# suvajit-patra/sl-hwgat

Hardware: AMD Instinct MI355X
Metric: clips/sec fwd+bwd at B=64 T=128 J=67; %HBM roofline; 1->8 GPU scaling (higher is better)
Workload: dtype f32

## Files before the change

### sl-hwgat_amd/csrc/gemm_f32.h

```cpp
#pragma once
#include "common.h"

struct NtArgs {
    const float* A; const float* W; const float* bias; float* C;
    float* C2; const float* res; const float* aux;
    const float* mean; const float* rstd; const float* gamma; const float* beta;
    int64_t M; int N, K;
    uint32_t pro_seed, epi_seed; float pro_p, epi_p;
    int64_t row0;
    float* stat_sum; float* stat_sq;
    int mg_F, mg_K;
    const uint32_t* seed_base;
};

struct MergeWalk {
    int k, f; int64_t b; int F, K, step;
    __device__ __forceinline__ void start(int64_t m, int F_, int K_, int step_) {
        F = F_; K = K_; step = step_;
        const uint32_t mm = (uint32_t)m, fr = mm / (uint32_t)K_;
        k = (int)(mm - fr * (uint32_t)K_);
        const uint32_t bb = fr / (uint32_t)F_;
        f = (int)(fr - bb * (uint32_t)F_);
        b = bb;
    }
    __device__ __forceinline__ int64_t mrow() const { return (b * (F >> 1) + (f >> 1)) * K + k; }
    __device__ __forceinline__ int64_t off(int N) const { return mrow() * (2 * (int64_t)N) + (int64_t)(f & 1) * N; }
    __device__ __forceinline__ void next() {
        k += step;
        const bool wk = k >= K;
        k -= wk ? K : 0;
        f += wk ? 1 : 0;
        const bool wf = f >= F;
        f -= wf ? F : 0;
        b += wf ? 1 : 0;
    }
};

struct TnArgs {
    const float* A; const float* B; float* dW; float* db;
    const float* mean; const float* rstd; const float* gamma; const float* beta;
    int64_t M; int N, K;
    int n_split; int64_t rows_per_split;
    uint32_t pro_seed; float pro_p;
    int64_t row0;
    const uint32_t* seed_base;
    float* det_dw; float* det_db; int det_cap;
};


int hwgat_launch_tn256(TnArgs a, hipStream_t st, float* ws = nullptr, int64_t ws_floats = 0);
int64_t hwgat_tn256_ws_floats(int64_t M, int N, int K);

int hwgat_launch_nt256(const NtArgs& a, int pro, int epi, hipStream_t st);
```

### sl-hwgat_amd/csrc/gemm_f32.hip

```cpp
#include <stdlib.h>
#include <type_traits>
#include "common.h"
#include "fused_ops.h"
#include "gemm_f32.h"
#include "gemm_tn64.h"

namespace {

constexpr int BK_MIN = 16;

using NtSmall = TileCfg<2, 2, 2, 2>;
using NtBig = TileCfg<4, 2, 2, 4, 32, 1>;
using NtK16 = TileCfg<2, 2, 2, 2, 16, 3>;
using NtN64 = TileCfg<4, 1, 1, 2>;

template <int PRO, int EPI, typename C, bool RAGGED = false, int STAT = 0>
__global__ __launch_bounds__(C::THREADS, C::OCC * C::THREADS / 256) void gemm_nt_k(NtArgs p) {
    HWGAT_RESOLVE_SEEDS2(p);
    constexpr int BM = C::BM, BN = C::BN, TMW = C::TMW, TNW = C::TNW, PA = C::PA, PW = C::PW, RPP = C::RPP;
    constexpr int BK = C::BK, LDT = C::LDT;
    __shared__ __attribute__((aligned(16))) float sm[2 * (BM + BN) * LDT];
    const int tid = threadIdx.x, lane = tid & 63, wave = tid >> 6;
    const int lq = lane & 31, hh = lane >> 5;
    const int wm = wave / C::WN, wn = wave % C::WN;
// ... 230 lines not shown
                        }
                    }
                    __builtin_amdgcn_fence(__ATOMIC_ACQ_REL, "wavefront");
                    __builtin_amdgcn_wave_barrier();
                }
            }
            if constexpr (STAT == X_STAT || STAT == X_STAT_MERGE) {
                __syncthreads();
                for (int q = tid; q < BM; q += C::THREADS) {
                    int64_t mr = m0 + q;
                    if constexpr (STAT == X_STAT_MERGE) { MergeWalk w; w.start(m0 + q, p.mg_F, p.mg_K, 1); mr = w.mrow(); }
                    atomicAdd(p.stat_sum + mr, rowstat[2 * q]);
                    atomicAdd(p.stat_sq + mr, rowstat[2 * q + 1]);
                }
            }
        }
        __syncthreads();
        t += gridDim.x;
        if (t >= n_tiles) break;
        m0 = mn; n0 = nn;
    }
}


using TnSmall = TileCfg<2, 2, 2, 2>;
using TnBig = TileCfg<4, 2, 2, 4, 32, 1>;
using TnK16 = TileCfg<2, 2, 2, 2, 16, 3>;

template <int PRO, bool BLN, typename C, bool MF16 = false, bool RAGGED = false>
__global__ __launch_bounds__(C::THREADS, C::OCC * C::THREADS / 256) void gemm_tn_k(TnArgs p) {
    HWGAT_RESOLVE_SEED1(p);
    constexpr int TM = C::BK;
    constexpr int BT = C::BM;
    constexpr int LDR = MF16 ? BT + 16 : BT;
    constexpr int TNW = C::TMW, TKW = C::TNW;
    constexpr int TPR = BT / 4;
    constexpr int RPP = C::THREADS / TPR;
    constexpr int NP = TM / RPP;
    __shared__ __attribute__((aligned(16))) float sm[2 * 2 * TM * LDR];
    const int tid = threadIdx.x, lane = tid & 63, wave = tid >> 6;
    const int lq = lane & 31, hh = lane >> 5;
    const int wn = wave / C::WN, wk = wave % C::WN;
    const int tiles_n = p.N / BT, tiles_k = p.K / BT, n_tiles = tiles_n * tiles_k;
    const int xcd = blockIdx.x & 7, j = blockIdx.x >> 3;
    const int tile = j % n_tiles;
    const int split = (j / n_tiles) * 8 + xcd;
    if (split >= p.n_split) return;
    const int n0 = (tile / tiles_k) * BT, k0 = (tile % tiles_k) * BT;
    const int64_t r_begin = (int64_t)split * p.rows_per_split;
    const int64_t r_end = r_begin + p.rows_per_split < p.M ? r_begin + p.rows_per_split : p.M;
    if (r_begin >= r_end) return;
    const int n_it = RAGGED ? (int)((r_end - r_begin + TM - 1) / TM) : (int)((r_end - r_begin) / TM);
    const int64_t m_last = p.M - 1;

    const int lrow = tid / TPR, lc4 = (tid % TPR) * 4;
    const uint32_t pro_th = drop_thresh(p.pro_p);
    const float pro_sc = 1.0f / (1.0f - p.pro_p);
    f32x4 ra[NP], rb[NP];
    float bm[NP], bs[NP];
    f32x4 colsum = {0.f, 0.f, 0.f, 0.f};
    f32x4 lg = {1.f, 1.f, 1.f, 1.f}, lb = {0.f, 0.f, 0.f, 0.f};
    if constexpr (BLN) {
        lg = *reinterpret_cast<const f32x4*>(p.gamma + k0 + lc4);
        lb = *reinterpret_cast<const f32x4*>(p.beta + k0 + lc4);
    }

    auto issue = [&](int it) {
        const int64_t r0 = r_begin + (int64_t)it * TM + lrow;
#pragma unroll
        for (int i = 0; i < NP; ++i) {
            int64_t row = r0 + RPP * i;
            if constexpr (RAGGED) row = row < m_last ? row : m_last;
            ra[i] = *reinterpret_cast<const f32x4*>(p.A + row * p.N + n0 + lc4);
            rb[i] = *reinterpret_cast<const f32x4*>(p.B + row * p.K + k0 + lc4);
            if constexpr (BLN) { bm[i] = p.mean[row]; bs[i] = p.rstd[row]; }
        }
    };
    auto commit = [&](int buf, int it) {
        float* As = sm + buf * (2 * TM * LDR);
        float* Bs = As + TM * LDR;
        const int64_t r0 = r_begin + (int64_t)it * TM + lrow;
#pragma unroll
        for (int i = 0; i < NP; ++i) {
            f32x4 a = ra[i], b = rb[i];
            if constexpr (PRO == PRO_DROP)
                a *= drop_keep4(p.pro_seed, (uint64_t)((RAGGED ? p.row0 : 0) + r0 + RPP * i) * p.N + n0 + lc4, pro_th, pro_sc);
            if constexpr (BLN) b = (b - bm[i]) * bs[i] * lg + lb;
            if constexpr (RAGGED) { if (r0 + RPP * i > m_last) a = f32x4{0.f, 0.f, 0.f, 0.f}; }
            colsum += a;
            *reinterpret_cast<f32x4*>(As + (lrow + RPP * i) * LDR + lc4) = a;
            *reinterpret_cast<f32x4*>(Bs + (lrow + RPP * i) * LDR + lc4) = b;
        }
    };

    constexpr int TI = MF16 ? TNW * 2 : TNW, TJ = MF16 ? TKW * 2 : TKW, TS = MF16 ? 16 : 32;
    typedef typename std::conditional<MF16, f32x4, f32x16>::type acc_t;
    acc_t acc[TI][TJ];
#pragma unroll
    for (int i = 0; i < TI; ++i)
#pragma unroll
        for (int jj = 0; jj < TJ; ++jj)
#pragma unroll
            for (int e = 0; e < (MF16 ? 4 : 16); ++e) acc[i][jj][e] = 0.f;

    issue(0);
    commit(0, 0);
    __syncthreads();
    int buf = 0;
    const int lc = MF16 ? (lane & 15) : lq, lk = MF16 ? (lane >> 4) : hh;
    constexpr int KPS = MF16 ? 4 : 2;
    for (int it = 0; it < n_it; ++it) {
        const bool have_next = it + 1 < n_it;
        if (have_next) issue(it + 1);
        const float* As = sm + buf * (2 * TM * LDR) + wn * (TNW * 32) + lc;
        const float* Bs = sm + buf * (2 * TM * LDR) + TM * LDR + wk * (TKW * 32) + lc;
        constexpr int NSTEP = TM / KPS, CH = MF16 ? 2 : 4, NCH = NSTEP / CH;
        float fa[2][CH][TI], fb[2][CH][TJ];
        auto fetch = [&](int c, int slot) {
#pragma unroll
            for (int e = 0; e < CH; ++e) {
                const int ro = (KPS * (c * CH + e) + lk) * LDR;
#pragma unroll
                for (int i = 0; i < TI; ++i) fa[slot][e][i] = As[ro + TS * i];
#pragma unroll
                for (int jj = 0; jj < TJ; ++jj) fb[slot][e][jj] = Bs[ro + TS * jj];
            }
        };
        fetch(0, 0);
#pragma unroll
        for (int c = 0; c < NCH; ++c) {
            if (c + 1 < NCH) fetch(c + 1, (c + 1) & 1);
            __builtin_amdgcn_sched_barrier(0);
#pragma unroll
            for (int e = 0; e < CH; ++e)
#pragma unroll
                for (int i = 0; i < TI; ++i)
#pragma unroll
                    for (int jj = 0; jj < TJ; ++jj) {
                        if constexpr (MF16)
                            acc[i][jj] = __builtin_amdgcn_mfma_f32_16x16x4f32(fa[c & 1][e][i], fb[c & 1][e][jj], acc[i][jj], 0, 0, 0);
                        else
                            acc[i][jj] = __builtin_amdgcn_mfma_f32_32x32x2f32(fa[c & 1][e][i], fb[c & 1][e][jj], acc[i][jj], 0, 0, 0);
                    }
            __builtin_amdgcn_sched_barrier(0);
        }
        if (have_next) commit(buf ^ 1, it + 1);
        __syncthreads();
        buf ^= 1;
    }
    const bool det = p.det_dw != nullptr;
    float* dwo = det ? p.det_dw + (int64_t)split * p.N * p.K : p.dW;
#pragma unroll
    for (int i = 0; i < TI; ++i)
#pragma unroll
        for (int jj = 0; jj < TJ; ++jj)
#pragma unroll
            for (int r = 0; r < (MF16 ? 4 : 16); ++r) {
                const int n = n0 + wn * (TNW * 32) + i * TS + (MF16 ? 4 * lk + r : crow(r, hh));
                const int k = k0 + wk * (TKW * 32) + jj * TS + lc;
                HWGAT_TN_ACC(det, dwo, (int64_t)n * p.K + k, acc[i][jj][r]);
            }
    if (p.db != nullptr && k0 == 0) {
        float* red = sm;
        __syncthreads();
        *reinterpret_cast<f32x4*>(red + lrow * BT + lc4) = colsum;
        __syncthreads();
        if (tid < BT) {
            float s = 0.f;
#pragma unroll
            for (int q = 0; q < RPP; ++q) s += red[q * BT + tid];
            HWGAT_TN_ACC(det, det ? p.det_db + (int64_t)split * p.N : p.db, n0 + tid, s);
        }
    }
}

__global__ void transpose_k(const float* __restrict__ in, float* __restrict__ out, int R, int C) {
    __shared__ float tile[32][33];
    const int c0 = blockIdx.x * 32, r0 = blockIdx.y * 32;
    for (int i = threadIdx.y; i < 32; i += 8)
        if (r0 + i < R && c0 + threadIdx.x < C) tile[i][threadIdx.x] = in[(int64_t)(r0 + i) * C + c0 + threadIdx.x];
    __syncthreads();
    for (int i = threadIdx.y; i < 32; i += 8)
        if (c0 + i < C && r0 + threadIdx.x < R) out[(int64_t)(c0 + i) * R + r0 + threadIdx.x] = tile[threadIdx.x][i];
}

template <int PRO, typename C, bool RAGGED = false>
int launch_nt(const NtArgs& a, int epi, hipStream_t st, bool fold = false) {
    const int64_t tiles = ((a.M + C::BM - 1) / C::BM) * (a.N / C::BN);
    const int grid = (int)(tiles < C::SLOTS ? tiles : C::SLOTS);
    if (fold) {
        if constexpr (PRO == PRO_NONE) {
            if (epi == EPI_BIAS) gemm_nt_k<PRO_NONE, EPI_BIAS, C, RAGGED, X_LNFOLD><<<grid, C::THREADS, 0, st>>>(a);
            else if (epi == EPI_BIAS_GELU_DROP) gemm_nt_k<PRO_NONE, EPI_BIAS_GELU_DROP, C, RAGGED, X_LNFOLD><<<grid, C::THREADS, 0, st>>>(a);
            else if (epi == EPI_BIAS_GELU_DROP_G) gemm_nt_k<PRO_NONE, EPI_BIAS_GELU_DROP_G, C, RAGGED, X_LNFOLD><<<grid, C::THREADS, 0, st>>>(a);
            else return HWGAT_EINVAL;
            HWGAT_LAUNCH_CHECK();
        }
        return HWGAT_EINVAL;
    }
    if (a.stat_sum != nullptr) {
        if constexpr (PRO == PRO_NONE && !RAGGED) {
            if (a.mg_K > 0) gemm_nt_k<PRO_NONE, EPI_BIAS_DROP_RES, C, false, 2><<<grid, C::THREADS, 0, st>>>(a);
            else gemm_nt_k<PRO_NONE, EPI_BIAS_DROP_RES, C, false, 1><<<grid, C::THREADS, 0, st>>>(a);
            HWGAT_LAUNCH_CHECK();
        }
        return HWGAT_EINVAL;
    }
    switch (epi) {
        case EPI_BIAS: gemm_nt_k<PRO, EPI_BIAS, C, RAGGED><<<grid, C::THREADS, 0, st>>>(a); break;
        case EPI_BIAS_DROP_RES: gemm_nt_k<PRO, EPI_BIAS_DROP_RES, C, RAGGED><<<grid, C::THREADS, 0, st>>>(a); break;
        case EPI_BIAS_GELU_DROP: gemm_nt_k<PRO, EPI_BIAS_GELU_DROP, C, RAGGED><<<grid, C::THREADS, 0, st>>>(a); break;
        case EPI_GELU_BWD: gemm_nt_k<PRO, EPI_GELU_BWD, C, RAGGED><<<grid, C::THREADS, 0, st>>>(a); break;
        case EPI_BIAS_GELU_DROP_G: gemm_nt_k<PRO, EPI_BIAS_GELU_DROP_G, C, RAGGED><<<grid, C::THREADS, 0, st>>>(a); break;
        case EPI_MUL_AUX: gemm_nt_k<PRO, EPI_MUL_AUX, C, RAGGED><<<grid, C::THREADS, 0, st>>>(a); break;
        case EPI_NONE: gemm_nt_k<PRO, EPI_NONE, C, RAGGED><<<grid, C::THREADS, 0, st>>>(a); break;
        case EPI_BIAS_RELU_DROP:
            if constexpr (PRO == PRO_NONE) { gemm_nt_k<PRO_NONE, EPI_BIAS_RELU_DROP, C, RAGGED><<<grid, C::THREADS, 0, st>>>(a); break; }
            return HWGAT_EINVAL;
        case EPI_RELU_BWD:
            if constexpr (PRO == PRO_NONE) { gemm_nt_k<PRO_NONE, EPI_RELU_BWD, C, RAGGED><<<grid, C::THREADS, 0, st>>>(a); break; }
            return HWGAT_EINVAL;
        default: return HWGAT_EINVAL;
    }
    HWGAT_LAUNCH_CHECK();
}

NtArgs nt_rows(NtArgs a, int64_t r0, int64_t rows) {
    a.A += r0 * a.K;
    a.C += r0 * a.N;
    if (a.C2) a.C2 += r0 * a.N;
    if (a.res) a.res += r0 * a.N;
    if (a.aux) a.aux += r0 * a.N;
    if (a.mean) { a.mean += r0; a.rstd += r0; }
    a.M = rows;
    a.row0 = r0;
    return a;
}
TnArgs tn_rows(TnArgs a, int64_t r0, int64_t rows) {
    a.A += r0 * a.N;
    a.B += r0 * a.K;
    if (a.mean) { a.mean += r0; a.rstd += r0; }
    a.M = rows;
    a.row0 = r0;
    return a;
}

int tile_override() {
    static const int v = [] {
        const char* e = lab_env("HWGAT_GEMM_TILE");
        return !e ? 0 : (e[0] == 's' ? 1 : (e[0] == 'b' ? 2 : (e[0] == 'k' ? 3 : (e[0] == 'm' ? 6 : (e[0] == 't' ? 7 : 0)))));
    }();
    return v;
}

int launch_nt_n64(const NtArgs& a, int pro, int epi, hipStream_t st) {
    const int64_t m_bulk = a.M / 128 * 128;
    if (m_bulk) {
        NtArgs b = a;
        b.M = m_bulk;
        int rc;
        switch (pro) {
            case PRO_NONE: rc = launch_nt<PRO_NONE, NtN64>(b, epi, st); break;
            case PRO_LN_FOLD: rc = launch_nt<PRO_NONE, NtN64>(b, epi, st, true); break;
            case PRO_LN: rc = launch_nt<PRO_LN, NtN64>(b, epi, st); break;
            case PRO_DROP: rc = launch_nt<PRO_DROP, NtN64>(b, epi, st); break;
            default: return HWGAT_EINVAL;
        }
        if (rc || m_bulk == a.M) return rc;
    }
    const NtArgs t = nt_rows(a, m_bulk, a.M - m_bulk);
    switch (pro) {
        case PRO_NONE: return launch_nt<PRO_NONE, NtN64, true>(t, epi, st);
        case PRO_LN: return launch_nt<PRO_LN, NtN64, true>(t, epi, st);
        case PRO_DROP: return launch_nt<PRO_DROP, NtN64, true>(t, epi, st);
        default: return HWGAT_EINVAL;
    }
}

template <int PRO, bool BLN, typename C, bool MF16 = false, bool RAGGED = false>
int launch_tn(TnArgs a, hipStream_t st) {
    constexpr int TM = C::BK;
    const int n_tiles = (a.N / C::BM) * (a.K / C::BM);
    auto gcd = [](int x, int y) { while (y) { int t = x % y; x = y; y = t; } return x; };
    const int r_min = n_tiles / gcd(n_tiles, C::SLOTS);
    static const int min_rounds = [] { const char* e = lab_env("HWGAT_TN_ROUNDS"); return e ? atoi(e) : 1; }();
    int r = r_min;
    while (r < min_rounds) r += r_min;
    int64_t want = (int64_t)C::SLOTS * r / n_tiles;
    const int64_t max_split = a.M / (TM * 16) > 0 ? a.M / (TM * 16) : 1;
    if (want > max_split) want = max_split;
    if (want < 1) want = 1;
    int64_t rows = (a.M + want - 1) / want;
    rows = (rows + TM - 1) / TM * TM;
    a.n_split = (int)((a.M + rows - 1) / rows);
    a.rows_per_split = rows;
    if (a.det_dw && a.n_split > a.det_cap) return HWGAT_ESHAPE;
    const int grid = ((a.n_split + 7) / 8) * 8 * n_tiles;
    gemm_tn_k<PRO, BLN, C, MF16, RAGGED><<<grid, C::THREADS, 0, st>>>(a);
    HWGAT_LAUNCH_CHECK();
}

}

extern "C" int hwgat_linear_nt_f32_ex(const float* A, const float* W, const float* bias, float* C, int64_t M,
                                      int N, int K, int pro, const float* mean, const float* rstd,
                                      const float* gamma, const float* beta, uint32_t pro_seed, float pro_p,
                                      int epi, const float* res, float* C2, const float* aux, uint32_t epi_seed,
                                      float epi_p, float* stat_sum, float* stat_sq, int merge_F, int merge_K,
                                      const uint32_t* seed_base, void* stream) {
    if (!A || !W || !C || M <= 0 || N <= 0 || K <= 0) return HWGAT_EINVAL;
    if (N % 64 || K % 32 || ((M + 127) / 128) * (int64_t)(N / 64) > 0x7fffffff) return HWGAT_ESHAPE;
    if ((pro == PRO_LN || pro == PRO_LN_FOLD) && (!mean || !rstd || !gamma || !beta)) return HWGAT_EINVAL;
    if (pro == PRO_LN_FOLD) {
        if (epi != EPI_BIAS && epi != EPI_BIAS_GELU_DROP && epi != EPI_BIAS_GELU_DROP_G) return HWGAT_EINVAL;
        if (M % 128) return HWGAT_ESHAPE;
    }
    if (epi == EPI_BIAS_DROP_RES && !res) return HWGAT_EINVAL;
    if ((epi == EPI_BIAS_GELU_DROP || epi == EPI_BIAS_GELU_DROP_G) && !C2) return HWGAT_EINVAL;
    if ((epi == EPI_GELU_BWD || epi == EPI_MUL_AUX || epi == EPI_RELU_BWD) && !aux) return HWGAT_EINVAL;
    if (pro_p < 0.f || pro_p >= 1.f || epi_p < 0.f || epi_p >= 1.f) return HWGAT_EINVAL;
    if (epi_is_relu(epi) && pro != PRO_NONE) return HWGAT_EINVAL;
    const bool stat = stat_sum != nullptr || stat_sq != nullptr || merge_K > 0;
    if (stat) {
        if (!stat_sum || !stat_sq || pro != PRO_NONE || epi != EPI_BIAS_DROP_RES) return HWGAT_EINVAL;
        if (M % 256) return HWGAT_ESHAPE;
        if (merge_K > 0 && (merge_F <= 0 || (merge_F & 1) || M % ((int64_t)merge_F * merge_K))) return HWGAT_EINVAL;
    }
    if (pro == PRO_DROP && pro_p == 0.f) pro = PRO_NONE;
    NtArgs a{A, W, bias, C, C2, res, aux, mean, rstd, gamma, beta, M, N, K, pro_seed, epi_seed, pro_p, epi_p, 0, stat_sum, stat_sq, merge_K > 0 ? merge_F : 0, merge_K > 0 ? merge_K : 0};
    a.seed_base = seed_base;
    hipStream_t st = (hipStream_t)stream;
    if (N % 128) {
        if (stat) return HWGAT_ESHAPE;
        return launch_nt_n64(a, pro, epi, st);
    }
    const int64_t m_bulk = M / 128 * 128;
    if (m_bulk != M) {
        if (m_bulk) {
            const int rc = hwgat_linear_nt_f32(A, W, bias, C, m_bulk, N, K, pro, mean, rstd, gamma, beta, pro_seed, pro_p,
                                               epi, res, C2, aux, epi_seed, epi_p, seed_base, stream);
            if (rc) return rc;
        }
        const NtArgs t = nt_rows(a, m_bulk, M - m_bulk);
        switch (pro) {
            case PRO_NONE: return launch_nt<PRO_NONE, NtSmall, true>(t, epi, st);
            case PRO_LN: return launch_nt<PRO_LN, NtSmall, true>(t, epi, st);
            case PRO_DROP: return launch_nt<PRO_DROP, NtSmall, true>(t, epi, st);
            default: return HWGAT_EINVAL;
        }
    }
    static const bool nt_old = [] { const char* e = lab_env("HWGAT_NT_KERNEL"); return e && e[0] == 'o'; }();
    static const int nt256_min_k = [] { const char* e = lab_env("HWGAT_NT256_MINK"); return e ? atoi(e) : 128; }();
    if (!nt_old && !epi_is_relu(epi) && tile_override() == 0 && N % 256 == 0 && K >= nt256_min_k && M >= 256 &&
        ((M / 256) * (N / 256) >= 128 || a.stat_sum != nullptr)) {
        const int64_t m256 = M / 256 * 256;
        NtArgs b = a;
        b.M = m256;
        const int rc = hwgat_launch_nt256(b, pro, epi, st);
        if (rc || m256 == M) return rc;
        const NtArgs t = nt_rows(a, m256, M - m256);
        switch (pro) {
            case PRO_NONE: return launch_nt<PRO_NONE, NtSmall, true>(t, epi, st);
            case PRO_LN_FOLD: return launch_nt<PRO_NONE, NtSmall, true>(t, epi, st, true);
            case PRO_LN: return launch_nt<PRO_LN, NtSmall, true>(t, epi, st);
            case PRO_DROP: return launch_nt<PRO_DROP, NtSmall, true>(t, epi, st);
            default: return HWGAT_EINVAL;
        }
    }
    const bool heavy = epi == EPI_BIAS_DROP_RES || epi == EPI_BIAS_GELU_DROP || epi == EPI_GELU_BWD || epi == EPI_BIAS_GELU_DROP_G || epi == EPI_MUL_AUX ||
                       epi_is_relu(epi);
    const bool big = tile_override() == 2 && (M % 256 == 0) && (N % 256 == 0);
    const bool k16 = tile_override() == 3 || (tile_override() == 0 && heavy);
#define NT_GO(P) return big ? launch_nt<P, NtBig>(a, epi, st) : (k16 ? launch_nt<P, NtK16>(a, epi, st) : launch_nt<P, NtSmall>(a, epi, st))
    switch (pro) {
        case PRO_NONE: NT_GO(PRO_NONE);
        case PRO_LN_FOLD: return k16 ? launch_nt<PRO_NONE, NtK16>(a, epi, st, true) : launch_nt<PRO_NONE, NtSmall>(a, epi, st, true);
        case PRO_LN: NT_GO(PRO_LN);
        case PRO_DROP: NT_GO(PRO_DROP);
        default: return HWGAT_EINVAL;
    }
#undef NT_GO
}

extern "C" int hwgat_linear_nt_f32(const float* A, const float* W, const float* bias, float* C, int64_t M,
                                   int N, int K, int pro, const float* mean, const float* rstd,
                                   const float* gamma, const float* beta, uint32_t pro_seed, float pro_p,
                                   int epi, const float* res, float* C2, const float* aux, uint32_t epi_seed,
                                   float epi_p, const uint32_t* seed_base, void* stream) {
    return hwgat_linear_nt_f32_ex(A, W, bias, C, M, N, K, pro, mean, rstd, gamma, beta, pro_seed, pro_p, epi, res, C2, aux,
                                  epi_seed, epi_p, nullptr, nullptr, 0, 0, seed_base, stream);
}

static bool tn256_takes(int64_t M, int N, int K, float pro_p, const float* mean) {
    const int ov = tile_override();
    return M % 32 == 0 && (ov == 0 || ov == 7) && N % 256 == 0 && K % 256 == 0 && (int64_t)N * K > 256 * 256 && !(pro_p > 0.f && mean);
}

extern "C" int64_t hwgat_linear_tn_f32_ws_bytes(int64_t M, int N, int K) {
    if (hwgat_tn64_takes(N, K)) return hwgat_tn64_ws_bytes(M, N, K);
    if (M <= 0 || N <= 0 || K <= 0 || !tn256_takes(M, N, K, 0.f, nullptr)) return 0;
    return hwgat_tn256_ws_floats(M, N, K) * 4;
}

extern "C" int hwgat_linear_tn_f32_ws(const float* A, const float* B, float* dW, float* db, int64_t M, int N,
                                      int K, uint32_t pro_seed, float pro_p, const float* mean,
                                      const float* rstd, const float* gamma, const float* beta, float* ws,
                                      int64_t ws_bytes, const uint32_t* seed_base, void* stream) {
    if (!A || !B || !dW || M <= 0 || N <= 0 || K <= 0) return HWGAT_EINVAL;
    if (mean && (!rstd || !gamma || !beta)) return HWGAT_EINVAL;
    if (pro_p < 0.f || pro_p >= 1.f) return HWGAT_EINVAL;
    if (hwgat_tn64_takes(N, K))
        return hwgat_tn64_run(HWGAT_F32, A, B, dW, db, M, N, K, pro_seed, pro_p, mean, rstd, gamma, beta, seed_base,
                              ws && ws_bytes >= hwgat_tn64_ws_bytes(M, N, K) ? ws : nullptr, ws_bytes, (hipStream_t)stream);
    if (ws && ws_bytes > 0 && N % 128 == 0 && K % 128 == 0 && tn256_takes(M, N, K, pro_p, mean)) {
        TnArgs a{A, B, dW, db, mean, rstd, gamma, beta, M, N, K, 0, 0, pro_seed, pro_p, 0};
        a.seed_base = seed_base;
        return hwgat_launch_tn256(a, (hipStream_t)stream, ws, ws_bytes / 4);
    }
    return hwgat_linear_tn_f32(A, B, dW, db, M, N, K, pro_seed, pro_p, mean, rstd, gamma, beta, seed_base, stream);
}

static int tn_f32_impl(const float* A, const float* B, float* dW, float* db, int64_t M, int N,
                       int K, uint32_t pro_seed, float pro_p, const float* mean,
                       const float* rstd, const float* gamma, const float* beta,
                       const uint32_t* seed_base, DetWs det, void* stream) {
    if (!A || !B || !dW || M <= 0 || N <= 0 || K <= 0) return HWGAT_EINVAL;
    if (mean && (!rstd || !gamma || !beta)) return HWGAT_EINVAL;
    if (N % 128 || K % 128) return HWGAT_ESHAPE;
    if (pro_p < 0.f || pro_p >= 1.f) return HWGAT_EINVAL;
    TnArgs a{A, B, dW, db, mean, rstd, gamma, beta, M, N, K, 0, 0, pro_seed, pro_p, 0};
    a.seed_base = seed_base;
    a.det_dw = det.dw; a.det_db = det.db; a.det_cap = det.cap;
    hipStream_t st = (hipStream_t)stream;
    const int64_t m_bulk = M / 32 * 32;
    if (m_bulk != M) {
        if (det.dw) return HWGAT_ESHAPE;
        if (m_bulk) {
            const int rc = hwgat_linear_tn_f32(A, B, dW, db, m_bulk, N, K, pro_seed, pro_p, mean, rstd, gamma, beta, seed_base, stream);
            if (rc) return rc;
        }
        const TnArgs t = tn_rows(a, m_bulk, M - m_bulk);
        if (pro_p > 0.f) return mean ? launch_tn<PRO_DROP, true, TnSmall, false, true>(t, st) : launch_tn<PRO_DROP, false, TnSmall, false, true>(t, st);
        return mean ? launch_tn<PRO_NONE, true, TnSmall, false, true>(t, st) : launch_tn<PRO_NONE, false, TnSmall, false, true>(t, st);
    }
    const int ov = tile_override();
    if ((ov == 0 || ov == 7) && N % 256 == 0 && K % 256 == 0 && (int64_t)N * K > 256 * 256 && !(pro_p > 0.f && mean))
        return hwgat_launch_tn256(a, st);
    const bool big = ov == 2 && (N % 256 == 0) && (K % 256 == 0);
    const bool k16 = ov == 3;
    const bool mf16 = ov == 6;
#define TN_GO(P, L) return mf16 ? launch_tn<P, L, TnSmall, true>(a, st) : (big ? launch_tn<P, L, TnBig>(a, st) : (k16 ? launch_tn<P, L, TnK16>(a, st) : launch_tn<P, L, TnSmall>(a, st)))
    if (pro_p > 0.f) { if (mean) TN_GO(PRO_DROP, true); else TN_GO(PRO_DROP, false); }
    if (mean) TN_GO(PRO_NONE, true);
    TN_GO(PRO_NONE, false);
#undef TN_GO
}

extern "C" int hwgat_linear_tn_f32(const float* A, const float* B, float* dW, float* db, int64_t M, int N,
                                   int K, uint32_t pro_seed, float pro_p, const float* mean,
                                   const float* rstd, const float* gamma, const float* beta,
                                   const uint32_t* seed_base, void* stream) {
    if (hwgat_tn64_takes(N, K))
        return hwgat_tn64_run(HWGAT_F32, A, B, dW, db, M, N, K, pro_seed, pro_p, mean, rstd, gamma, beta, seed_base,
                              nullptr, 0, (hipStream_t)stream);
    return tn_f32_impl(A, B, dW, db, M, N, K, pro_seed, pro_p, mean, rstd, gamma, beta, seed_base, DetWs{nullptr, nullptr, 0}, stream);
}

namespace {
__global__ __launch_bounds__(256) void tn_det_reduce_k(const float* __restrict__ ws, float* __restrict__ out, int cap, int64_t stride,
                                                       int64_t count) {
    const int64_t i = (int64_t)blockIdx.x * 256 + threadIdx.x;
    if (i >= count) return;
    float s = 0.f;
    int sp = 0;
    for (; sp + 8 <= cap; sp += 8) {
        float v[8];
#pragma unroll
        for (int j = 0; j < 8; ++j) v[j] = ws[(sp + j) * stride + i];
#pragma unroll
        for (int j = 0; j < 8; ++j) s += v[j];
    }
    for (; sp < cap; ++sp) s += ws[sp * stride + i];
    out[i] += s;
}
}
int hwgat_tn_det_reduce(const float* ws, float* out, int cap, int64_t stride, int64_t count, hipStream_t st) {
    tn_det_reduce_k<<<(unsigned)((count + 255) / 256), 256, 0, st>>>(ws, out, cap, stride, count);
    HWGAT_LAUNCH_CHECK();
}

static int64_t tn_det_cap(int64_t M, int N, int K) {
    auto gcd = [](int64_t x, int64_t y) { while (y) { int64_t t = x % y; x = y; y = t; } return x; };
    const int64_t t128 = (int64_t)(N / 128) * (K / 128);
    int64_t cap = 0;
    for (int64_t slots : {512, 768, 1024}) {
        const int64_t r = t128 / gcd(t128, slots);
        cap = cap > slots * r / t128 ? cap : slots * r / t128;
    }
    if (N % 256 == 0 && K % 256 == 0) {
        const int64_t t256 = (int64_t)(N / 256) * (K / 256), r = t256 / gcd(t256, 256);
        const int64_t w = 256 * r / t256 > 8 ? 256 * r / t256 : 8;
        cap = cap > w ? cap : w;
    }
    const int64_t by_rows = M / 32 + 1;
    cap = cap < by_rows ? cap : by_rows;
    return cap + 8;
}
extern "C" int64_t hwgat_linear_tn_det_bytes(int64_t M, int N, int K) {
    if (hwgat_tn64_takes(N, K)) return hwgat_tn64_ws_bytes(M, N, K);
    if (M <= 0 || N <= 0 || K <= 0 || N % 128 || K % 128) return 0;
    return tn_det_cap(M, N, K) * ((int64_t)N * K + N) * 4;
}

extern "C" int hwgat_linear_tn_f32_det(const float* A, const float* B, float* dW, float* db, int64_t M, int N,
                                       int K, uint32_t pro_seed, float pro_p, const float* mean,
                                       const float* rstd, const float* gamma, const float* beta,
                                       const uint32_t* seed_base, float* ws, int64_t ws_bytes, void* stream) {
    if (!ws || N <= 0 || K <= 0) return HWGAT_EINVAL;
    if (hwgat_tn64_takes(N, K))
        return hwgat_tn64_run(HWGAT_F32, A, B, dW, db, M, N, K, pro_seed, pro_p, mean, rstd, gamma, beta, seed_base, ws,
                              ws_bytes, (hipStream_t)stream);
    const int64_t per = (int64_t)N * K + N;
    const int64_t cap = ws_bytes / 4 / per;
    if (cap < 1) return HWGAT_ESHAPE;
    const DetWs det{ws, ws + cap * (int64_t)N * K, (int)(cap > 0x7fffffff ? 0x7fffffff : cap)};
    int rc = tn_f32_impl(A, B, dW, db, M, N, K, pro_seed, pro_p, mean, rstd, gamma, beta, seed_base, det, stream);
    if (rc) return rc;
    rc = hwgat_tn_det_reduce(det.dw, dW, det.cap, (int64_t)N * K, (int64_t)N * K, (hipStream_t)stream);
    if (rc || !db) return rc;
    return hwgat_tn_det_reduce(det.db, db, det.cap, N, N, (hipStream_t)stream);
}

extern "C" int hwgat_transpose_f32(const float* in, float* out, int R, int C, void* stream) {
    if (!in || !out || R <= 0 || C <= 0) return HWGAT_EINVAL;
    dim3 grid((C + 31) / 32, (R + 31) / 32), block(32, 8);
    transpose_k<<<grid, block, 0, (hipStream_t)stream>>>(in, out, R, C);
    HWGAT_LAUNCH_CHECK();
}

__global__ void drop_mask_k(float* out, int64_t n, uint32_t seed, float p, const uint32_t* seed_base) {
    seed += seed_base_of(seed_base);
    const uint32_t th = drop_thresh(p);
    const float sc = 1.0f / (1.0f - p);
    for (int64_t i = (int64_t)blockIdx.x * 256 + threadIdx.x; i < n; i += (int64_t)gridDim.x * 256)
        out[i] = drop_keep(seed, (uint64_t)i, th, sc);
}
extern "C" int hwgat_dropout_mask_f32(float* out, int64_t n, uint32_t seed, float p, const uint32_t* seed_base, void* stream) {
    if (!out || n <= 0 || p < 0.f || p >= 1.f) return HWGAT_EINVAL;
    const int grid = (int)((n + 255) / 256 < 2048 ? (n + 255) / 256 : 2048);
    drop_mask_k<<<grid, 256, 0, (hipStream_t)stream>>>(out, n, seed, p, seed_base);
    HWGAT_LAUNCH_CHECK();
}
```

Baseline: 636.7.

## Add persistent NT GEMM kernel with direct buffer-to-LDS loads

Adds a new 256x256 f32 NT GEMM kernel that stages A and W tiles straight into LDS with buffer_load...lds, double-buffers them, and interleaves the next slab's loads with MFMA work under pinned scheduling groups. The kernel is persistent with a grid capped at 256, so it prefetches the next tile during the current tile's epilogue and prefetches epilogue operands (residual, aux, LN stats) early. The dispatcher routes large-K shapes to it through a heuristic, with an env override. The aim is to hide global load latency and cut VGPR staging, at the cost of a large fixed LDS footprint (one block per CU) and complex hand scheduling.

```diff
diff --git a/sl-hwgat_amd/csrc/gemm_f32.h b/sl-hwgat_amd/csrc/gemm_f32.h
--- a/sl-hwgat_amd/csrc/gemm_f32.h
+++ b/sl-hwgat_amd/csrc/gemm_f32.h
@@ -52,3 +52,6 @@
 int64_t hwgat_tn256_ws_floats(int64_t M, int N, int K);
 
 int hwgat_launch_nt256(const NtArgs& a, int pro, int epi, hipStream_t st);
+
+bool hwgat_nt256d_takes(const NtArgs& a, int pro, int epi);
+int hwgat_launch_nt256d(const NtArgs& a, int pro, int epi, hipStream_t st);
diff --git a/sl-hwgat_amd/csrc/gemm_f32.hip b/sl-hwgat_amd/csrc/gemm_f32.hip
--- a/sl-hwgat_amd/csrc/gemm_f32.hip
+++ b/sl-hwgat_amd/csrc/gemm_f32.hip
@@ -556,6 +556,12 @@
 
 }
 
+static bool nt256d_wins(int N, int K) {
+    if (K < 512) return false;
+    if (N == 256 && K > 512) return false;
+    return true;
+}
+
 extern "C" int hwgat_linear_nt_f32_ex(const float* A, const float* W, const float* bias, float* C, int64_t M,
                                       int N, int K, int pro, const float* mean, const float* rstd,
                                       const float* gamma, const float* beta, uint32_t pro_seed, float pro_p,
@@ -605,12 +611,16 @@
     }
     static const bool nt_old = [] { const char* e = lab_env("HWGAT_NT_KERNEL"); return e && e[0] == 'o'; }();
     static const int nt256_min_k = [] { const char* e = lab_env("HWGAT_NT256_MINK"); return e ? atoi(e) : 128; }();
-    if (!nt_old && !epi_is_relu(epi) && tile_override() == 0 && N % 256 == 0 && K >= nt256_min_k && M >= 256 &&
-        ((M / 256) * (N / 256) >= 128 || a.stat_sum != nullptr)) {
-        const int64_t m256 = M / 256 * 256;
-        NtArgs b = a;
-        b.M = m256;
-        const int rc = hwgat_launch_nt256(b, pro, epi, st);
+    const char* nt_force = lab_env("HWGAT_NT_KERNEL");
+    const bool force_reg = nt_force && nt_force[0] == 'r', force_dma = nt_force && nt_force[0] == 'd';
+    const bool wide = !nt_old && !epi_is_relu(epi) && tile_override() == 0 && N % 256 == 0 && M >= 256 &&
+                      ((M / 256) * (N / 256) >= 128 || a.stat_sum != nullptr);
+    const int64_t m256 = M / 256 * 256;
+    NtArgs b = a;
+    b.M = m256;
+    const bool dma = wide && !force_reg && hwgat_nt256d_takes(b, pro, epi) && (force_dma || nt256d_wins(N, K));
+    if (wide && (K >= nt256_min_k || dma)) {
+        const int rc = dma ? hwgat_launch_nt256d(b, pro, epi, st) : hwgat_launch_nt256(b, pro, epi, st);
         if (rc || m256 == M) return rc;
         const NtArgs t = nt_rows(a, m256, M - m256);
         switch (pro) {
diff --git a/sl-hwgat_amd/csrc/gemm_f32_nt256d.hip b/sl-hwgat_amd/csrc/gemm_f32_nt256d.hip
--- /dev/null
+++ b/sl-hwgat_amd/csrc/gemm_f32_nt256d.hip
@@ -0,0 +1,401 @@
+#include <type_traits>
+#include <utility>
+#include "common.h"
+#include "fused_ops.h"
+#include "gemm_f32.h"
+
+namespace {
+
+constexpr int BT = 256, BK = 32;
+constexpr int ROWB = BK * 4;
+constexpr int OPB = BT * ROWB;
+constexpr int BUFB = 2 * OPB;
+constexpr int STG_OFF = 2 * BUFB;
+constexpr int STG_WAVE = 7168;
+constexpr int SINK_OFF = 4096;
+constexpr int STAT_OFF = STG_OFF + 4 * STG_WAVE;
+constexpr int SMEM = STAT_OFF + 2 * BT * 2 * 4;
+static_assert(SMEM == 160 * 1024, "LDS budget");
+constexpr int NDMA = 16;
+
+constexpr int SG_MFMA = 0x008, SG_VMEM = 0x010, SG_DS_RD = 0x100;
+
+typedef __attribute__((address_space(3))) void* lds_ptr_t;
+
+template <int N> __device__ __forceinline__ void wait_vm() { asm volatile("s_waitcnt vmcnt(%0)" ::"n"(N < 63 ? N : 63) : "memory"); }
+__device__ __forceinline__ void wait_lds() { asm volatile("s_waitcnt lgkmcnt(0)" ::: "memory"); }
+__device__ __forceinline__ void wg_barrier() {
+    __builtin_amdgcn_sched_barrier(0);
+    __builtin_amdgcn_s_barrier();
+    __builtin_amdgcn_sched_barrier(0);
+}
+__device__ __forceinline__ f32x4 ld16_counted(const float* p) {
+    f32x4 v;
+    asm volatile("global_load_dwordx4 %0, %1, off" : "=&v"(v) : "v"(p) : "memory");
+    return v;
+}
+template <int OFF> __device__ __forceinline__ float ld4_counted(const float* p) {
+    float v;
+    asm volatile("global_load_dword %0, %1, off offset:%2" : "=&v"(v) : "v"(p), "n"(OFF * 4) : "memory");
+    return v;
+}
+__device__ __forceinline__ void hold(f32x4& v) { asm volatile("" : "+v"(v)::"memory"); }
+__device__ __forceinline__ void hold(float& v) { asm volatile("" : "+v"(v)::"memory"); }
+
+template <class F, int... I>
+__device__ __forceinline__ void for_each_const(F&& f, std::integer_sequence<int, I...>) { (f(std::integral_constant<int, I>{}), ...); }
+
+template <int G, int M1, int N1, int M2 = 0, int N2 = 0>
+__device__ __forceinline__ void pin() {
+#pragma unroll
+    for (int q = 0; q < G; ++q) {
+        __builtin_amdgcn_sched_group_barrier(SG_MFMA, 64 / G, 0);
+        if constexpr (N1 > 0) __builtin_amdgcn_sched_group_barrier(M1, N1, 0);
+        if constexpr (N2 > 0) __builtin_amdgcn_sched_group_barrier(M2, N2, 0);
+    }
+}
+
+#ifdef HWGAT_LAB
+__device__ unsigned long long* g_nt256d_stamps = nullptr;
+#define NT256D_STAMP(i) do { if (g_nt256d_stamps && threadIdx.x == 0) g_nt256d_stamps[blockIdx.x * 2 + (i)] = __builtin_amdgcn_s_memtime(); } while (0)
+#else
+#define NT256D_STAMP(i) do {} while (0)
+#endif
+
+template <int EPI, int STAT>
+__global__ __launch_bounds__(256, 1) void gemm_nt256d_k(NtArgs p) {
+    HWGAT_RESOLVE_SEEDS2(p);
+    __shared__ __attribute__((aligned(16))) unsigned char smb[SMEM];
+    const int tid = threadIdx.x, lane = tid & 63;
+    const int wave = __builtin_amdgcn_readfirstlane(tid >> 6);
+    const int lq = lane & 31, hh = lane >> 5;
+    const int wm = wave >> 1, wn = wave & 1;
+    const int tiles_n = p.N / BT;
+    const int row_blocks = (int)(p.M / BT);
+    const int n_tiles = row_blocks * tiles_n;
+    const int n_slab = p.K / BK;
+    const int K4 = p.K * 4;
+
+    const int swz_tiles = (row_blocks / 8) * 8 * tiles_n;
+    auto tile_origin = [&](int t, int64_t& m0, int& n0) {
+        int rb, nt;
+        if (t < swz_tiles) {
+            rb = (t / (8 * tiles_n)) * 8 + (t & 7);
+            nt = (t >> 3) % tiles_n;
+        } else {
+            const int w = t - swz_tiles;
+            rb = (row_blocks / 8) * 8 + w / tiles_n;
+            nt = w % tiles_n;
+        }
+        m0 = (int64_t)rb * BT;
+        n0 = nt * BT;
+    };
+
+    const int voff0 = (lane >> 3) * K4 + (((lane & 7) ^ (lane >> 4)) << 4);
+    const int voff1 = voff0 ^ 64;
+    auto stage_piece = [&](int j, int buf, __amdgpu_buffer_rsrc_t ra, __amdgpu_buffer_rsrc_t rw, int kb, bool live) {
+        const int r = wave * 64 + j * 8;
+        const int sink = STG_OFF + wave * STG_WAVE + SINK_OFF;
+        const int da = live ? buf * BUFB + r * ROWB : sink, dw = live ? buf * BUFB + OPB + r * ROWB : sink;
+        __builtin_amdgcn_raw_ptr_buffer_load_lds(ra, (lds_ptr_t)(smb + da), 16, (j & 1) ? voff1 : voff0, r * K4 + kb, 0, 0);
+        __builtin_amdgcn_raw_ptr_buffer_load_lds(rw, (lds_ptr_t)(smb + dw), 16, (j & 1) ? voff1 : voff0, r * K4 + kb, 0, 0);
+    };
+    auto stage = [&](int buf, __amdgpu_buffer_rsrc_t ra, __amdgpu_buffer_rsrc_t rw, int kb, bool live) {
+#pragma unroll
+        for (int j = 0; j < 8; ++j) stage_piece(j, buf, ra, rw, kb, live);
+    };
+    const __amdgpu_buffer_rsrc_t rnull = __builtin_amdgcn_make_buffer_rsrc((void*)p.A, 0, 0, 0x00020000);
+    auto rsrc_a = [&](int64_t m0) {
+        return __builtin_amdgcn_make_buffer_rsrc((void*)(p.A + m0 * p.K), 0, 0x7fffffff, 0x00020000);
+    };
+    auto rsrc_w = [&](int n0) {
+        return __builtin_amdgcn_make_buffer_rsrc((void*)(p.W + (int64_t)n0 * p.K), 0, 0x7fffffff, 0x00020000);
+    };
+
+    int aoff[4], woff[4];
+#pragma unroll
+    for (int kk = 0; kk < 4; ++kk) {
+        const int ch = ((2 * kk + hh) ^ ((lq >> 1) & 7)) << 4;
+        aoff[kk] = (wm * 128 + lq) * ROWB + ch;
+        woff[kk] = OPB + (wn * 128 + lq) * ROWB + ch;
+    }
+    f32x16 acc[4][4];
+    struct Frag { f32x4 a[4], b[4]; };
+    Frag f0, f1;
+    auto fetch = [&](Frag& f, int buf, int kk) {
+        const unsigned char* base = smb + buf * BUFB;
+#pragma unroll
+        for (int i = 0; i < 4; ++i) {
+            f.a[i] = *reinterpret_cast<const f32x4*>(base + aoff[kk] + i * 32 * ROWB);
+            f.b[i] = *reinterpret_cast<const f32x4*>(base + woff[kk] + i * 32 * ROWB);
+        }
+    };
+    auto mfma64 = [&](const Frag& f) {
+#pragma unroll
+        for (int e = 0; e < 4; ++e)
+#pragma unroll
+            for (int i = 0; i < 4; ++i)
+#pragma unroll
+                for (int j = 0; j < 4; ++j)
+                    acc[i][j] = __builtin_amdgcn_mfma_f32_32x32x2f32(f.a[i][e], f.b[j][e], acc[i][j], 0, 0, 0);
+    };
+
+    constexpr bool EXTRA = epi_reads_extra(EPI);
+    constexpr int LP = (EXTRA ? 4 : 0) + (STAT == X_LNFOLD ? 8 : 0);
+    constexpr int SP = (EPI == EPI_BIAS_GELU_DROP || EPI == EPI_BIAS_GELU_DROP_G) ? 8 : 4;
+    constexpr int NSTW = 15 * LP + 16 * SP + NDMA;
+    constexpr int NPRE = LP + (STAT == X_LNFOLD ? 2 : 0);
+    const int er = lane >> 5, ec = (lane & 31) * 4;
+    const int64_t rs2 = 2 * (int64_t)p.N;
+    f32x4 ex[2][4];
+    float rr[2][4], rm[2][4];
+    f32x4 bv, sv, cv;
+    const float* exq = nullptr; const float* rq = nullptr; const float* mq = nullptr;
+    auto request = [&](auto pc_tag, int b) {
+        constexpr int pc = decltype(pc_tag)::value;
+        if constexpr (EXTRA) {
+#pragma unroll
+            for (int ps = 0; ps < 4; ++ps) { ex[b][ps] = ld16_counted(exq); exq += rs2; }
+        }
+        if constexpr (STAT == X_LNFOLD) {
+            rr[b][0] = ld4_counted<pc * 8 + 0>(rq); rm[b][0] = ld4_counted<pc * 8 + 0>(mq);
+            rr[b][1] = ld4_counted<pc * 8 + 2>(rq); rm[b][1] = ld4_counted<pc * 8 + 2>(mq);
+            rr[b][2] = ld4_counted<pc * 8 + 4>(rq); rm[b][2] = ld4_counted<pc * 8 + 4>(mq);
+            rr[b][3] = ld4_counted<pc * 8 + 6>(rq); rm[b][3] = ld4_counted<pc * 8 + 6>(mq);
+        }
+    };
+    auto hold_piece = [&](int b) {
+        if constexpr (EXTRA) {
+#pragma unroll
+            for (int ps = 0; ps < 4; ++ps) hold(ex[b][ps]);
+        }
+        if constexpr (STAT == X_LNFOLD) {
+#pragma unroll
+            for (int ps = 0; ps < 4; ++ps) { hold(rr[b][ps]); hold(rm[b][ps]); }
+        }
+    };
+
+    int t = blockIdx.x;
+    if (t >= n_tiles) return;
+    int64_t m0; int n0;
+    tile_origin(t, m0, n0);
+    __amdgpu_buffer_rsrc_t xc = rsrc_a(m0), wc = rsrc_w(n0), xn = xc, wnx = wc;
+    NT256D_STAMP(0);
+    stage(0, xc, wc, 0, true);
+    stage(1, xc, wc, ROWB, true);
+    wait_vm<0>();
+    wg_barrier();
+    int buf = 0;
+
+    while (true) {
+#pragma unroll
+        for (int i = 0; i < 4; ++i)
+#pragma unroll
+            for (int j = 0; j < 4; ++j)
+#pragma unroll
+                for (int e = 0; e < 16; ++e) acc[i][j][e] = 0.f;
+
+        const int tn = t + gridDim.x;
+        const bool more = tn < n_tiles;
+        int64_t mn = m0; int nn = n0;
+        if (more) { tile_origin(tn, mn, nn); xn = rsrc_a(mn); wnx = rsrc_w(nn); }
+
+#pragma clang loop unroll(disable)
+        for (int sl = 0; sl < n_slab; ++sl) {
+            int s = sl;
+            asm volatile("" : "+s"(s));
+            const bool last = s + 1 == n_slab;
+            fetch(f0, buf, 0);
+            {
+                const bool live = s > 0 && (!last || more);
+                __amdgpu_buffer_rsrc_t ra = last ? xn : xc, rw = last ? wnx : wc;
+                if (!live) { ra = rnull; rw = rnull; }
+                const unsigned char* fb = smb + buf * BUFB;
+                const int kb = last ? 0 : (s + 1) * ROWB;
+#pragma unroll
+                for (int g = 0; g < 16; ++g) {
+                    const int e = g >> 2, i = g & 3;
+#pragma unroll
+                    for (int j = 0; j < 4; ++j)
+                        acc[i][j] = __builtin_amdgcn_mfma_f32_32x32x2f32(f0.a[i][e], f0.b[j][e], acc[i][j], 0, 0, 0);
+                    if (g < 4) f1.a[g] = *reinterpret_cast<const f32x4*>(fb + aoff[1] + g * 32 * ROWB);
+                    else if (g < 8) f1.b[g - 4] = *reinterpret_cast<const f32x4*>(fb + woff[1] + (g - 4) * 32 * ROWB);
+                    else stage_piece(g - 8, buf ^ 1, ra, rw, kb, live);
+                    __builtin_amdgcn_sched_barrier(0);
+                }
+            }
+            __builtin_amdgcn_sched_barrier(0);
+            fetch(f0, buf, 2);
+            mfma64(f1);
+            pin<8, SG_DS_RD, 1>();
+            __builtin_amdgcn_sched_barrier(0);
+            fetch(f1, buf, 3);
+            mfma64(f0);
+            pin<8, SG_DS_RD, 1>();
+            __builtin_amdgcn_sched_barrier(0);
+            if (last) {
+                const int col = n0 + wn * 128 + ec;
+                bv = f32x4{0.f, 0.f, 0.f, 0.f};
+                if constexpr (epi_has_bias(EPI) && STAT != X_LNFOLD)
+                    if (p.bias) bv = ld16_counted(p.bias + col);
+                if constexpr (STAT == X_LNFOLD) { sv = ld16_counted(p.gamma + col); cv = ld16_counted(p.beta + col); }
+                const int64_t r0 = m0 + wm * 128 + er;
+                if constexpr (EXTRA) exq = (EPI == EPI_BIAS_DROP_RES ? p.res : p.aux) + r0 * p.N + col;
+                if constexpr (STAT == X_LNFOLD) { rq = p.rstd + r0; mq = p.mean + r0; }
+                request(std::integral_constant<int, 0>{}, 0);
+            }
+            __builtin_amdgcn_sched_barrier(0);
+            mfma64(f1);
+            __builtin_amdgcn_sched_barrier(0);
+            if (last) wait_vm<NPRE>();
+            else if (s == 0) wait_vm<NSTW>();
+            else wait_vm<0>();
+            wait_lds();
+            wg_barrier();
+            buf ^= 1;
+        }
+        if (more) stage(buf ^ 1, xn, wnx, ROWB, true);
+        __builtin_amdgcn_sched_barrier(0);
+
+        {
+            const uint32_t epi_th = drop_thresh(p.epi_p);
+            const float epi_sc = 1.0f / (1.0f - p.epi_p);
+            float* stg = reinterpret_cast<float*>(smb + STG_OFF + wave * STG_WAVE);
+            float* rowstat = reinterpret_cast<float*>(smb + STAT_OFF);
+            const int col = n0 + wn * 128 + ec;
+            MergeWalk mw;
+            if constexpr (STAT == X_STAT_MERGE) mw.start(m0 + wm * 128 + er, p.mg_F, p.mg_K, 2);
+            int64_t off = (m0 + wm * 128 + er) * p.N + col;
+            auto piece = [&](auto pc_tag) {
+                constexpr int pc = decltype(pc_tag)::value;
+                constexpr int i = pc >> 2, q = pc & 3, b = pc & 1;
+                if constexpr (pc + 1 < 16) request(std::integral_constant<int, pc + 1>{}, b ^ 1);
+                if constexpr (pc == 0) {
+                    if constexpr (LP > 0 || epi_has_bias(EPI)) {
+                        if (more) wait_vm<NDMA + LP>(); else wait_vm<LP>();
+                        hold(bv);
+                        if constexpr (STAT == X_LNFOLD) { hold(sv); hold(cv); }
+                    }
+                } else if constexpr (LP > 0) {
+                    if (pc < 15) wait_vm<SP + LP>(); else wait_vm<SP>();
+                }
+                hold_piece(b);
+#pragma unroll
+                for (int j = 0; j < 4; ++j)
+#pragma unroll
+                    for (int r = 0; r < 4; ++r) stg[(4 * hh + r) * 128 + j * 32 + lq] = acc[i][j][4 * q + r];
+                __builtin_amdgcn_fence(__ATOMIC_ACQ_REL, "wavefront");
+                __builtin_amdgcn_wave_barrier();
+#pragma unroll
+                for (int ps = 0; ps < 4; ++ps) {
+                    const int lr = wm * 128 + pc * 8 + 2 * ps + er;
+                    f32x4 v = *reinterpret_cast<const f32x4*>(stg + (2 * ps + er) * 128 + ec);
+                    if constexpr (STAT == X_LNFOLD) v = v * rr[b][ps] + (cv - sv * (rm[b][ps] * rr[b][ps]));
+                    else v += bv;
+                    f32x4 dk = {1.f, 1.f, 1.f, 1.f};
+                    if constexpr (epi_drops(EPI)) {
+                        dk = drop_keep4(p.epi_seed, (uint64_t)off, epi_th, epi_sc);
+                    }
+                    if constexpr (EPI == EPI_BIAS_DROP_RES) {
+                        v = ex[b][ps] + v * dk;
+                    } else if constexpr (EPI == EPI_BIAS_GELU_DROP) {
+                        *reinterpret_cast<f32x4*>(p.C2 + off) = v;
+                        v.x = gelu_f(v.x) * dk.x; v.y = gelu_f(v.y) * dk.y;
+                        v.z = gelu_f(v.z) * dk.z; v.w = gelu_f(v.w) * dk.w;
+                    } else if constexpr (EPI == EPI_BIAS_GELU_DROP_G) {
+                        float u4[4] = {v.x, v.y, v.z, v.w}, g4[4];
+                        const float k4[4] = {dk.x, dk.y, dk.z, dk.w};
+#pragma unroll
+                        for (int e = 0; e < 4; ++e) gelu_fwd_grad(u4[e], k4[e], u4[e], g4[e]);
+                        v = f32x4{u4[0], u4[1], u4[2], u4[3]};
+                        const f32x4 gq = {g4[0], g4[1], g4[2], g4[3]};
+                        *reinterpret_cast<f32x4*>(p.C2 + off) = gq;
+                    } else if constexpr (EPI == EPI_MUL_AUX) {
+                        v *= ex[b][ps];
+                    } else if constexpr (EPI == EPI_GELU_BWD) {
+                        const f32x4 h = ex[b][ps];
+                        v.x *= dk.x * gelu_grad(h.x); v.y *= dk.y * gelu_grad(h.y);
+                        v.z *= dk.z * gelu_grad(h.z); v.w *= dk.w * gelu_grad(h.w);
+                    }
+                    if constexpr (STAT == X_STAT || STAT == X_STAT_MERGE) {
+                        float s1 = (v.x + v.y) + (v.z + v.w), s2 = (v.x * v.x + v.y * v.y) + (v.z * v.z + v.w * v.w);
+                        s1 = group_sum<32>(s1); s2 = group_sum<32>(s2);
+                        if ((lane & 31) == 0) { f32x2 st = {s1, s2}; *reinterpret_cast<f32x2*>(rowstat + (wn * BT + lr) * 2) = st; }
+                        if constexpr (STAT == X_STAT_MERGE) {
+                            *reinterpret_cast<f32x4*>(p.C + mw.off(p.N) + col) = v;
+                            mw.next();
+                        } else {
+                            *reinterpret_cast<f32x4*>(p.C + off) = v;
+                        }
+                    } else {
+                        *reinterpret_cast<f32x4*>(p.C + off) = v;
+                    }
+                    off += rs2;
+                }
+                __builtin_amdgcn_fence(__ATOMIC_ACQ_REL, "wavefront");
+                __builtin_amdgcn_wave_barrier();
+                __builtin_amdgcn_sched_barrier(0);
+            };
+            for_each_const(piece, std::make_integer_sequence<int, 16>{});
+            if constexpr (STAT == X_STAT || STAT == X_STAT_MERGE) {
+                wait_lds();
+                wg_barrier();
+                int64_t mr = m0 + tid;
+                if constexpr (STAT == X_STAT_MERGE) { MergeWalk w; w.start(m0 + tid, p.mg_F, p.mg_K, 1); mr = w.mrow(); }
+                atomicAdd(p.stat_sum + mr, rowstat[2 * tid] + rowstat[2 * (BT + tid)]);
+                atomicAdd(p.stat_sq + mr, rowstat[2 * tid + 1] + rowstat[2 * (BT + tid) + 1]);
+            }
+        }
+        t = tn;
+        if (!more) break;
+        m0 = mn; n0 = nn; xc = xn; wc = wnx;
+    }
+    NT256D_STAMP(1);
+}
+
+template <int EPI, int STAT>
+int go(const NtArgs& a, int grid, hipStream_t st) {
+    gemm_nt256d_k<EPI, STAT><<<grid, 256, 0, st>>>(a);
+    HWGAT_LAUNCH_CHECK();
+}
+
+}
+
+bool hwgat_nt256d_takes(const NtArgs& a, int pro, int epi) {
+    if (a.M % BT || a.N % BT || a.K % BK || a.M < BT || a.K < 3 * BK) return false;
+    if ((int64_t)BT * a.K * 4 > 0x3fffffff) return false;
+    if ((a.M / BT) * (a.N / BT) > 0x7fffffff) return false;
+    if (pro != PRO_NONE && pro != PRO_LN_FOLD) return false;
+    if (a.stat_sum != nullptr) return pro == PRO_NONE && epi == EPI_BIAS_DROP_RES;
+    if (pro == PRO_LN_FOLD) return epi == EPI_BIAS || epi == EPI_BIAS_GELU_DROP || epi == EPI_BIAS_GELU_DROP_G;
+    return epi == EPI_NONE || epi == EPI_BIAS || epi == EPI_BIAS_DROP_RES || epi == EPI_BIAS_GELU_DROP || epi == EPI_GELU_BWD ||
+           epi == EPI_BIAS_GELU_DROP_G || epi == EPI_MUL_AUX;
+}
+
+int hwgat_launch_nt256d(const NtArgs& a, int pro, int epi, hipStream_t st) {
+    if (!hwgat_nt256d_takes(a, pro, epi)) return HWGAT_ESHAPE;
+    const int64_t tiles = (a.M / BT) * (a.N / BT);
+    const int grid = (int)(tiles < 256 ? tiles : 256);
+    if (a.stat_sum != nullptr) return a.mg_K > 0 ? go<EPI_BIAS_DROP_RES, X_STAT_MERGE>(a, grid, st) : go<EPI_BIAS_DROP_RES, X_STAT>(a, grid, st);
+    if (pro == PRO_LN_FOLD) {
+        if (epi == EPI_BIAS) return go<EPI_BIAS, X_LNFOLD>(a, grid, st);
+        if (epi == EPI_BIAS_GELU_DROP) return go<EPI_BIAS_GELU_DROP, X_LNFOLD>(a, grid, st);
+        return go<EPI_BIAS_GELU_DROP_G, X_LNFOLD>(a, grid, st);
+    }
+    switch (epi) {
+        case EPI_BIAS: return go<EPI_BIAS, X_NONE>(a, grid, st);
+        case EPI_BIAS_DROP_RES: return go<EPI_BIAS_DROP_RES, X_NONE>(a, grid, st);
+        case EPI_BIAS_GELU_DROP: return go<EPI_BIAS_GELU_DROP, X_NONE>(a, grid, st);
+        case EPI_GELU_BWD: return go<EPI_GELU_BWD, X_NONE>(a, grid, st);
+        case EPI_BIAS_GELU_DROP_G: return go<EPI_BIAS_GELU_DROP_G, X_NONE>(a, grid, st);
+        case EPI_MUL_AUX: return go<EPI_MUL_AUX, X_NONE>(a, grid, st);
+        case EPI_NONE: return go<EPI_NONE, X_NONE>(a, grid, st);
+        default: return HWGAT_EINVAL;
+    }
+}
+
+#ifdef HWGAT_LAB
+extern "C" int hwgat_lab_nt256d_stamps(void* buf) {
+    return hipMemcpyToSymbol(HIP_SYMBOL(g_nt256d_stamps), &buf, sizeof(buf)) == hipSuccess ? 0 : HWGAT_EINVAL;
+}
+#endif
```

Result: no change. 641.8, median of 6 (+0.8%).
